# PantoMatrix/PantoMatrix

Measured on NVIDIA H100. Metric: motion_frames_per_sec, higher is better.
Workload: dtype fp16x3 (two fp16 operand planes, 3 products, f32 accumulate)

## Files before the change

### include/pm_emage.h

```cpp
#ifndef PM_EMAGE_H
#define PM_EMAGE_H
#include <stdint.h>
#ifdef __cplusplus
extern "C" {
#endif

#define PM_ABI_VERSION 6
#define PM_FMT_F16 0x100
#define PM_TC_TILE_SHIFT 16
int pm_abi_version(void);
int pm_memset_async(void* ptr, int value, long long bytes, void* stream);
int pm_device_cc(void);

int pm_tapgemm_f32(const float* A, long long a_bs, int lda, int batch, int rows_in, int cin,
                   const float* W, const float* bias, int taps, int stride, int pad,
                   int rows_out, int cout,
                   const float* residual, long long r_bs, int ldr,
                   int act, float slope,
                   float* out, long long o_bs, int ldo, void* stream);

int pm_tapgemm_tc(const uint16_t* A, long long a_ps, long long a_bs, int lda, int batch, int rows_in, int cin,
                  const uint16_t* W, long long w_ps, int w_rows, int ldw, int taps, int pad, int nsplit,
                  const float* bias, int rows_out, int cout,
                  const float* residual, long long r_bs, int ldr,
                  int act, int act_cols, float slope, float acc_scale,
                  float* out_f32, long long o_bs, int ldo,
                  uint16_t* out_bf16, long long ob_ps, long long ob_bs, int ldob, int out_nsplit,
                  const void* prefetch, long long prefetch_bytes, void* stream);

int pm_split_bf16(const float* x, long long x_bs, int ldx, int batch, int rows, int ch,
                  uint16_t* out, long long o_ps, long long o_bs, int ldo, int nsplit, void* stream);

// ... 114 lines not shown
```

### pantomatrix_b200/csrc/pm_common.cuh

```cuda
#pragma once
#include <cuda_bf16.h>
#include <cuda_fp16.h>
#include <cuda_runtime.h>
#include <stdint.h>

#define PM_OK 0
#define PM_EBADARG (-1)
#define PM_EUNSUPPORTED (-2)

#define PM_LAUNCH_CHECK()                                  \
  do {                                                     \
    cudaError_t _e = cudaGetLastError();                   \
    return _e == cudaSuccess ? PM_OK : (int)_e;            \
  } while (0)

#define PM_REQUIRE(cond) \
  do {                   \
    if (!(cond)) return PM_EBADARG; \
  } while (0)

static inline int pm_cdiv(long long a, long long b) { return (int)((a + b - 1) / b); }

static inline bool pm_first_use_on_device(unsigned long long& mask) {
  int d = 0;
// ... 37 lines not shown
  int nsplit;
};

__device__ __forceinline__ void pm_split3(float v, __nv_bfloat16 (&p)[3]) {
  p[0] = __float2bfloat16_rn(v);
  float r = v - __bfloat162float(p[0]);
  p[1] = __float2bfloat16_rn(r);
  r -= __bfloat162float(p[1]);
  p[2] = __float2bfloat16_rn(r);
}

#ifndef PM_FMT_F16
#define PM_FMT_F16 0x100
#endif
#define PM_F16_ACT_SCALE 64.0f
#define PM_TAKE_FMT(nsplit_var, flag_var)                          \
  const bool flag_var = ((nsplit_var) & PM_FMT_F16) != 0;          \
  (nsplit_var) &= 0xff

__device__ __forceinline__ float pm_f16_head(float v) {
  return __uint_as_float((__float_as_uint(v) + 0x00001000u) & 0xFFFFE000u);
}

template <bool F16>
__device__ __forceinline__ void pm_store_planes_t(const PmPlanes& P, long long row, int c, float v) {
  if constexpr (F16) {
    __half* o = reinterpret_cast<__half*>(P.ptr) + row * P.ld + c;
    v *= PM_F16_ACT_SCALE;
    if (P.nsplit <= 2) {
      const float f0 = P.nsplit == 2 ? pm_f16_head(v) : v;
      o[0] = __float2half_rn(f0);
      if (P.nsplit == 2) o[P.ps] = __float2half_rn(v - f0);
    } else {
      for (int pl = 0; pl < P.nsplit; ++pl) {
        const __half h = __float2half_rn(v);
        o[(long long)pl * P.ps] = h;
        v -= __half2float(h);
      }
    }
  } else {
    __nv_bfloat16* o = P.ptr + row * P.ld + c;
    for (int pl = 0; pl < P.nsplit; ++pl) {
      const __nv_bfloat16 h = __float2bfloat16_rn(v);
      o[(long long)pl * P.ps] = h;
      v -= __bfloat162float(h);
    }
  }
}
__device__ __forceinline__ void pm_store_planes(const PmPlanes& P, long long row, int c, float v) {
  pm_store_planes_t<false>(P, row, c, v);
}

template <bool F16>
__device__ __forceinline__ void pm_store_planes4_t(const PmPlanes& P, long long row, int c, float4 v) {
  if constexpr (F16) {
    __half* o = reinterpret_cast<__half*>(P.ptr) + row * P.ld + c;
    v.x *= PM_F16_ACT_SCALE; v.y *= PM_F16_ACT_SCALE; v.z *= PM_F16_ACT_SCALE; v.w *= PM_F16_ACT_SCALE;
    if (P.nsplit == 2) {
      const float4 f = make_float4(pm_f16_head(v.x), pm_f16_head(v.y), pm_f16_head(v.z), pm_f16_head(v.w));
      const __half2 a0 = __floats2half2_rn(f.x, f.y), a1 = __floats2half2_rn(f.z, f.w);
      const __half2 b0 = __floats2half2_rn(v.x - f.x, v.y - f.y), b1 = __floats2half2_rn(v.z - f.z, v.w - f.w);
      uint2 w0, w1;
      w0.x = *reinterpret_cast<const uint32_t*>(&a0); w0.y = *reinterpret_cast<const uint32_t*>(&a1);
      w1.x = *reinterpret_cast<const uint32_t*>(&b0); w1.y = *reinterpret_cast<const uint32_t*>(&b1);
      *reinterpret_cast<uint2*>(o) = w0;
      *reinterpret_cast<uint2*>(o + P.ps) = w1;
      return;
    }
    for (int pl = 0; pl < P.nsplit; ++pl) {
      const __half2 lo = __floats2half2_rn(v.x, v.y), hi = __floats2half2_rn(v.z, v.w);
      uint2 w;
      w.x = *reinterpret_cast<const uint32_t*>(&lo);
      w.y = *reinterpret_cast<const uint32_t*>(&hi);
      *reinterpret_cast<uint2*>(o + (long long)pl * P.ps) = w;
      v.x -= __low2float(lo); v.y -= __high2float(lo); v.z -= __low2float(hi); v.w -= __high2float(hi);
    }
  } else {
    __nv_bfloat16* o = P.ptr + row * P.ld + c;
    for (int pl = 0; pl < P.nsplit; ++pl) {
      const __nv_bfloat162 lo = __floats2bfloat162_rn(v.x, v.y), hi = __floats2bfloat162_rn(v.z, v.w);
      uint2 w;
      w.x = *reinterpret_cast<const uint32_t*>(&lo);
      w.y = *reinterpret_cast<const uint32_t*>(&hi);
      *reinterpret_cast<uint2*>(o + (long long)pl * P.ps) = w;
      v.x -= __low2float(lo); v.y -= __high2float(lo); v.z -= __low2float(hi); v.w -= __high2float(hi);
    }
  }
}
__device__ __forceinline__ void pm_store_planes4(const PmPlanes& P, long long row, int c, float4 v) {
  pm_store_planes4_t<false>(P, row, c, v);
}

static inline bool pm_planes_ok(const void* ptr, long long ps, int ld, int nsplit, int ch, bool vec4) {
  if (!ptr) return true;
  if (nsplit < 1 || nsplit > 3 || ld < ch) return false;
  if (vec4 && ((ld & 3) || (ps & 3) || (reinterpret_cast<uintptr_t>(ptr) & 7))) return false;
  return true;
}
```

### pantomatrix_b200/csrc/pm_tapgemm_tc.cu

```cuda
#include <cuda.h>
#include <stdio.h>
#include <stdlib.h>

#include <cstring>
#include "pm_common.cuh"
#include "../../include/pm_emage.h"


namespace {

constexpr int BM = 128;
constexpr int BK = 64;
constexpr int MMA_K = 16;
constexpr int A_TILE_BYTES = BM * BK * 2;
constexpr int PRODUCER_THREADS = 128;
constexpr int CONSUMER_THREADS = 256;
constexpr int NUM_THREADS = PRODUCER_THREADS + CONSUMER_THREADS;
constexpr int PRODUCER_REGS = 40, CONSUMER_REGS = 232;
static_assert(PRODUCER_THREADS * PRODUCER_REGS + CONSUMER_THREADS * CONSUMER_REGS == (65536 / NUM_THREADS & ~7) * NUM_THREADS,
              "the setmaxnreg split must use exactly the launch's register pool");
constexpr int STAMP_WARP = PRODUCER_THREADS / 32;
constexpr int MAX_STAGES = 8;
constexpr int RING_KB = 200;

struct TcParams {
  int taps, pad, nsplit, kblocks;
  int rows_out, cout, batch;
  int R, NB;
  int w_rows;
  const float* bias;
  const float* residual; long long r_bs; int ldr;
  int res_tma;
  int act, act_cols; float slope;
  float* out_f32; long long o_bs; int ldo;
  __nv_bfloat16* out_bf16; long long ob_ps, ob_bs; int ldob; int out_nsplit;
  int stages;
  int res_slot0, rot;
  const uint8_t* prefetch; long long prefetch_bytes;
  float acc_scale;
};

#ifdef PM_TC_TIMING
__device__ unsigned long long pm_tc_stamps[4096 * 8];
#define PM_STAMP(i)                                                                                              \
  do {                                                                                                           \
    if ((threadIdx.x & 31) == 0) {                                                                               \
      const unsigned cta_ = (blockIdx.z * gridDim.y + blockIdx.y) * gridDim.x + blockIdx.x;                      \
      if (cta_ < 4096) pm_tc_stamps[cta_ * 8 + (i)] = (unsigned long long)clock64();                             \
    }                                                                                                            \
  } while (0)
#else
#define PM_STAMP(i) do {} while (0)
#endif

#include "pm_tc_ptx.cuh"
// ... 10 lines not shown
  constexpr uint64_t A_PL = A_TILE_BYTES >> 4, W_PL = (BN * BK * 2) >> 4, K_ST = (MMA_K * 2) >> 4;
  if constexpr (NSPLIT == 3) {
#pragma unroll
    for (int k = 0; k < BK / MMA_K; ++k) mma_k16<BN, F16>(corr, a0 + k * K_ST, w0 + 2 * W_PL + k * K_ST);
#pragma unroll
    for (int k = 0; k < BK / MMA_K; ++k) mma_k16<BN, F16>(corr, a0 + A_PL + k * K_ST, w0 + W_PL + k * K_ST);
#pragma unroll
    for (int k = 0; k < BK / MMA_K; ++k) mma_k16<BN, F16>(corr, a0 + 2 * A_PL + k * K_ST, w0 + k * K_ST);
  }
  if constexpr (NSPLIT >= 2) {
#pragma unroll
    for (int k = 0; k < BK / MMA_K; ++k) mma_k16<BN, F16>(corr, a0 + k * K_ST, w0 + W_PL + k * K_ST);
#pragma unroll
    for (int k = 0; k < BK / MMA_K; ++k) mma_k16<BN, F16>(corr, a0 + A_PL + k * K_ST, w0 + k * K_ST);
  }
#pragma unroll
  for (int k = 0; k < BK / MMA_K; ++k) mma_k16<BN, F16>(main, a0 + k * K_ST, w0 + k * K_ST);
}

template <int BN, bool F16, int NSPLIT>
__global__ void __launch_bounds__(NUM_THREADS, 1) tapgemm_tc_kernel(const __grid_constant__ CUtensorMap map_a,
                                                                  const __grid_constant__ CUtensorMap map_w,
                                                                  const __grid_constant__ CUtensorMap map_r,
                                                                  const TcParams p) {
  constexpr int W_TILE_BYTES = BN * BK * 2;
  constexpr int NACC = BN / 2;
  constexpr int ST = BN + 8;
  constexpr int RES_BYTES = BM * BN * 4;

  extern __shared__ __align__(1024) uint8_t smem_raw[];
  uint8_t* tiles = reinterpret_cast<uint8_t*>((reinterpret_cast<uintptr_t>(smem_raw) + 1023) & ~uintptr_t(1023));
  const int stage_bytes = p.nsplit * (A_TILE_BYTES + W_TILE_BYTES);
  const int ring_bytes = p.stages * stage_bytes > BM * ST * 4 ? p.stages * stage_bytes : BM * ST * 4;
  uint64_t* bars = reinterpret_cast<uint64_t*>(tiles + ring_bytes);
  uint64_t* full_bar = bars;
  uint64_t* empty_bar = bars + MAX_STAGES;
  uint64_t* epi_bar = bars + 2 * MAX_STAGES;
  float* bias_s = reinterpret_cast<float*>(bars + 2 * MAX_STAGES + 2);

  const int warp = threadIdx.x >> 5, lane = threadIdx.x & 31;
  if (warp == STAMP_WARP) PM_STAMP(0);
  const int l0 = blockIdx.x * p.R;
  const int n0 = blockIdx.y * BN;
  const int b0 = blockIdx.z * p.NB;
  const int n_iter = p.taps * p.kblocks;

  if (threadIdx.x == 0) {
    asm volatile("prefetch.tensormap [%0];" ::"l"(&map_a) : "memory");
    asm volatile("prefetch.tensormap [%0];" ::"l"(&map_w) : "memory");
    if (p.res_tma) asm volatile("prefetch.tensormap [%0];" ::"l"(&map_r) : "memory");
    for (int s = 0; s < p.stages; ++s) {
      mbar_init(smem_u32(&full_bar[s]), 1);
      mbar_init(smem_u32(&empty_bar[s]), 2);
    }
    mbar_init(smem_u32(epi_bar), p.res_tma ? 2 : 1);
    asm volatile("fence.mbarrier_init.release.cluster;" ::: "memory");
  }
  __syncthreads();
  if (warp == STAMP_WARP) PM_STAMP(1);

  if (warp < PRODUCER_THREADS / 32) {
    setmaxnreg_dec<PRODUCER_REGS>();
    if (warp == 1 && lane == 0 && p.prefetch) {
      const long long ncta = (long long)gridDim.x * gridDim.y * gridDim.z;
      const long long cta = ((long long)blockIdx.z * gridDim.y + blockIdx.y) * gridDim.x + blockIdx.x;
      long long share = ((p.prefetch_bytes + ncta - 1) / ncta + 127) & ~127LL;
      long long off = cta * share;
      long long end = off + share < p.prefetch_bytes ? off + share : p.prefetch_bytes;
      end &= ~15LL;
      for (; off < end; off += 16384) {
        const uint32_t n = (uint32_t)(end - off < 16384 ? end - off : 16384);
        asm volatile("cp.async.bulk.prefetch.L2.global [%0], %1;" ::"l"(p.prefetch + off), "r"(n) : "memory");
      }
// ... 11 lines not shown
      mbar_wait_fast(smem_u32(&empty_bar[s]), ph ^ 1u);
      if (elect_one()) {
        const uint32_t bar = smem_u32(&full_bar[s]);
        uint8_t* st = tiles + (size_t)q * stage_bytes;
        mbar_expect_tx(bar, tx);
        for (int pl = 0; pl < p.nsplit; ++pl) {
          tma_load_4d(smem_u32(st + pl * A_TILE_BYTES), &map_a, bar, kb * BK, l0 + tap - p.pad, b0, pl);
          tma_load_3d(smem_u32(st + p.nsplit * A_TILE_BYTES + pl * W_TILE_BYTES), &map_w, bar, kb * BK, tap * p.w_rows + n0, pl);
        }
      }
      __syncwarp();
      if (++s == p.stages) { s = 0; ph ^= 1u; }
      if (++q == p.stages) q = 0;
      if (++kb == p.kblocks) { kb = 0; ++tap; }
    }
    if (p.res_tma) {
      for (int j = p.res_slot0; j < p.stages; ++j) {
        mbar_wait_fast(smem_u32(&empty_bar[s]), ph ^ 1u);
        if (++s == p.stages) { s = 0; ph ^= 1u; }
      }
      if (elect_one()) {
        const uint32_t bar = smem_u32(epi_bar);
        mbar_expect_tx(bar, (uint32_t)RES_BYTES);
        tma_load_3d(smem_u32(tiles + ring_bytes - RES_BYTES), &map_r, bar, n0, l0, b0);
      }
      __syncwarp();
    }
    return;
  }

  setmaxnreg_inc<CONSUMER_REGS>();
  const int ct = threadIdx.x - PRODUCER_THREADS;
  const int wg = ct >> 7;
  float acc0[NACC], acc1[NACC], accc[NACC];
#pragma unroll
  for (int i = 0; i < NACC; ++i) { acc0[i] = 0.f; acc1[i] = 0.f; accc[i] = 0.f; }
  {
    const uint32_t tiles_u32 = smem_u32(tiles);
    int s = 0, q = p.rot;
    uint32_t ph = 0;
    int prev = -1;
    auto kblock = [&](float (&main)[NACC]) {
      mbar_wait_fast(smem_u32(&full_bar[s]), ph);
      if (prev < 0 && warp == STAMP_WARP) PM_STAMP(2);
      const uint32_t a_base = tiles_u32 + (uint32_t)q * (uint32_t)stage_bytes + (uint32_t)wg * (64 * 128);
      const uint32_t w_base = tiles_u32 + (uint32_t)q * (uint32_t)stage_bytes + (uint32_t)(NSPLIT * A_TILE_BYTES);
      wgmma_fence();
      mma_kblock<BN, F16, NSPLIT>(main, accc, gmma_desc(GMMA_DESC_K_SW128, a_base), gmma_desc(GMMA_DESC_K_SW128, w_base));
      wgmma_commit();
      wgmma_wait<1>();
      if (prev >= 0 && ct % 128 == 0) mbar_arrive(smem_u32(&empty_bar[prev]));
      prev = s;
      if (++s == p.stages) { s = 0; ph ^= 1u; }
      if (++q == p.stages) q = 0;
    };
    int it = 0;
    for (; it + 1 < n_iter; it += 2) {
      kblock(acc0);
      kblock(acc1);
    }
    if (it < n_iter) kblock(acc0);
    if (warp == STAMP_WARP) PM_STAMP(3);
    wgmma_wait<0>();
    if (warp == STAMP_WARP) PM_STAMP(4);
    wgmma_fence_regs(acc0);
    wgmma_fence_regs(acc1);
    wgmma_fence_regs(accc);
  }
  named_bar_sync(1, CONSUMER_THREADS);
  {
    const int wq = warp & 3, t4 = lane & 3;
    const int r0 = wg * 64 + wq * 16 + (lane >> 2);
    float* stg = reinterpret_cast<float*>(tiles);
#pragma unroll
    for (int i = 0; i < NACC / 4; ++i) {
      const int c = 8 * i + 2 * t4;
#pragma unroll
      for (int h = 0; h < 2; ++h) {
        float v0 = acc0[4 * i + 2 * h] + acc1[4 * i + 2 * h];
        float v1 = acc0[4 * i + 2 * h + 1] + acc1[4 * i + 2 * h + 1];
        v0 += accc[4 * i + 2 * h];
        v1 += accc[4 * i + 2 * h + 1];
        if constexpr (F16) { v0 *= p.acc_scale; v1 *= p.acc_scale; }
        *reinterpret_cast<float2*>(stg + (r0 + 8 * h) * ST + c) = make_float2(v0, v1);
      }
    }
  }
  named_bar_sync(1, CONSUMER_THREADS);

  const bool vec_f = p.out_f32 && ((p.ldo & 3) == 0) && ((reinterpret_cast<uintptr_t>(p.out_f32) & 15) == 0) && ((p.o_bs & 3) == 0);
  const bool vec_b = p.out_bf16 && ((p.ldob & 3) == 0) && ((reinterpret_cast<uintptr_t>(p.out_bf16) & 7) == 0) &&
                     ((p.ob_bs & 3) == 0) && ((p.ob_ps & 3) == 0);
// ... 58 lines not shown
                                                         long long o_bs, int ldo, int nsplit) {
  const int b = blockIdx.y;
  const float* __restrict__ xb = x + (long long)b * x_bs;
  __nv_bfloat16* __restrict__ ob = out + (long long)b * o_bs;
  if (VEC) {
    const int ch4 = ch >> 2;
    const long long total = (long long)rows * ch4;
    for (long long i = (long long)blockIdx.x * blockDim.x + threadIdx.x; i < total; i += (long long)gridDim.x * blockDim.x) {
      const int r = (int)(i / ch4), c4 = (int)(i - (long long)r * ch4);
      const float4 v = *reinterpret_cast<const float4*>(xb + (long long)r * ldx + 4 * c4);
      const PmPlanes P{ob, o_ps, ldo, nsplit};
      pm_store_planes4_t<F16>(P, r, 4 * c4, v);
    }
  } else {
    const long long total = (long long)rows * ch;
    for (long long i = (long long)blockIdx.x * blockDim.x + threadIdx.x; i < total; i += (long long)gridDim.x * blockDim.x) {
      const int r = (int)(i / ch), c = (int)(i - (long long)r * ch);
      const PmPlanes P{ob, o_ps, ldo, nsplit};
      pm_store_planes_t<F16>(P, r, c, xb[(long long)r * ldx + c]);
    }
  }
}

template <int BN, bool F16, int NSPLIT>
int launch(const CUtensorMap& ma, const CUtensorMap& mw, const CUtensorMap& mr, TcParams& p, dim3 grid, cudaStream_t st) {
  constexpr int stage_bytes = NSPLIT * (A_TILE_BYTES + BN * BK * 2);
  constexpr int stages = RING_KB * 1024 / stage_bytes < MAX_STAGES ? RING_KB * 1024 / stage_bytes : MAX_STAGES;
  static_assert(stages >= 2, "the operand ring needs two stages");
  constexpr int staging = BM * (BN + 8) * 4, res_bytes = BM * BN * 4;
  static_assert(staging + res_bytes <= stages * stage_bytes && res_bytes <= (stages - 1) * stage_bytes,
                "staging and residual tiles must fit the ring side by side");
  p.stages = stages;
  p.res_slot0 = (stages * stage_bytes - res_bytes) / stage_bytes;
  p.rot = (p.res_slot0 - 1 - (p.taps * p.kblocks - 1) % stages + stages) % stages;
  const size_t smem = (size_t)stages * stage_bytes + 1024  + (2 * MAX_STAGES + 2) * sizeof(uint64_t) + BN * sizeof(float);
  static unsigned long long configured = 0;
  if (pm_first_use_on_device(configured)) {
    cudaError_t e = cudaFuncSetAttribute(tapgemm_tc_kernel<BN, F16, NSPLIT>, cudaFuncAttributeMaxDynamicSharedMemorySize, 227 * 1024);
    if (e != cudaSuccess) { configured = 0; return (int)e; }
  }
  tapgemm_tc_kernel<BN, F16, NSPLIT><<<grid, NUM_THREADS, smem, st>>>(ma, mw, mr, p);
  PM_LAUNCH_CHECK();
}

template <int BN>
int launch_fmt(const CUtensorMap& ma, const CUtensorMap& mw, const CUtensorMap& mr, TcParams& p, dim3 grid, cudaStream_t st,
               bool f16) {
  if (f16) {
    if (p.nsplit == 1) return launch<BN, true, 1>(ma, mw, mr, p, grid, st);
    if (p.nsplit == 2) return launch<BN, true, 2>(ma, mw, mr, p, grid, st);
    return launch<BN, true, 3>(ma, mw, mr, p, grid, st);
  }
  if (p.nsplit == 1) return launch<BN, false, 1>(ma, mw, mr, p, grid, st);
  if (p.nsplit == 2) return launch<BN, false, 2>(ma, mw, mr, p, grid, st);
  return launch<BN, false, 3>(ma, mw, mr, p, grid, st);
}

int pick_bn(long long row_tiles, int cout, int w_rows, int sms) {
  if (cout <= 64 || w_rows % 128) return 64;
  const long long waves64 = (row_tiles * pm_cdiv(cout, 64) + sms - 1) / sms;
  const long long waves128 = (row_tiles * pm_cdiv(cout, 128) + sms - 1) / sms;
  return waves128 * 14 <= waves64 * 10 ? 128 : 64;
}

}

extern "C" int pm_tapgemm_tc(const uint16_t* A, long long a_ps, long long a_bs, int lda, int batch, int rows_in, int cin,
                             const uint16_t* W, long long w_ps, int w_rows, int ldw, int taps, int pad, int nsplit,
                             const float* bias, int rows_out, int cout,
                             const float* residual, long long r_bs, int ldr,
                             int act, int act_cols, float slope, float acc_scale,
                             float* out_f32, long long o_bs, int ldo,
                             uint16_t* out_bf16, long long ob_ps, long long ob_bs, int ldob, int out_nsplit,
                             const void* prefetch, long long prefetch_bytes, void* stream) {
  PM_REQUIRE(A && W && (out_f32 || out_bf16));
  const int tile = (nsplit >> PM_TC_TILE_SHIFT) & 0xff;
  PM_TAKE_FMT(nsplit, f16);
  PM_TAKE_FMT(out_nsplit, out_f16);
  PM_REQUIRE(!out_bf16 || out_f16 == f16);
  PM_REQUIRE(f16 || acc_scale == 1.0f);
  PM_REQUIRE(!prefetch || (prefetch_bytes >= 0 && (reinterpret_cast<uintptr_t>(prefetch) & 15) == 0));
  PM_REQUIRE(batch > 0 && rows_in > 0 && rows_out > 0 && cin > 0 && cout > 0 && taps > 0);
  PM_REQUIRE(nsplit >= 1 && nsplit <= 3 && (!out_bf16 || (out_nsplit >= 1 && out_nsplit <= 3)));
  PM_REQUIRE(act >= PM_ACT_NONE && act <= PM_ACT_LEAKY);
  PM_REQUIRE((reinterpret_cast<uintptr_t>(A) & 15) == 0 && (reinterpret_cast<uintptr_t>(W) & 15) == 0);
  PM_REQUIRE((lda & 7) == 0 && (ldw & 7) == 0 && lda >= cin && ldw >= cin && w_rows >= cout);
  PM_REQUIRE(batch == 1 || (a_bs & 7) == 0);
  PM_REQUIRE(nsplit == 1 || ((a_ps & 7) == 0 && (w_ps & 7) == 0));
  PM_REQUIRE(!out_f32 || ldo >= cout);
  PM_REQUIRE(!out_bf16 || ldob >= cout);
  PM_REQUIRE(!residual || ldr >= cout);

  int R = 128;
  if (rows_out <= 64 && batch > 1) { R = 16; while (R < rows_out) R <<= 1; }
  const int NB = 128 / R;
  PM_REQUIRE(tile <= 2 && w_rows % 64 == 0 && (tile != 2 || w_rows % 128 == 0));
  int BNsel = tile == 1 ? 64 : 128;
  if (tile == 0) {
    int dev = 0, sms = 0;
    cudaError_t e = cudaGetDevice(&dev);
    if (e == cudaSuccess) e = cudaDeviceGetAttribute(&sms, cudaDevAttrMultiProcessorCount, dev);
    if (e != cudaSuccess) return (int)e;
    BNsel = pick_bn((long long)pm_cdiv(rows_out, R) * pm_cdiv(batch, NB), cout, w_rows, sms);
  }

  TcParams p;
  p.taps = taps; p.pad = pad; p.nsplit = nsplit; p.kblocks = (cin + BK - 1) / BK;
  p.rows_out = rows_out; p.cout = cout; p.batch = batch; p.R = R; p.NB = NB; p.w_rows = w_rows;
  p.bias = bias; p.residual = residual; p.r_bs = r_bs; p.ldr = ldr;
  p.act = act; p.act_cols = act_cols <= 0 ? cout : act_cols; p.slope = slope;
  p.out_f32 = out_f32; p.o_bs = o_bs; p.ldo = ldo;
  p.out_bf16 = reinterpret_cast<__nv_bfloat16*>(out_bf16); p.ob_ps = ob_ps; p.ob_bs = ob_bs; p.ldob = ldob;
  p.out_nsplit = out_bf16 ? out_nsplit : 0;
  p.stages = 0;
  p.prefetch = static_cast<const uint8_t*>(prefetch);
  p.prefetch_bytes = prefetch ? prefetch_bytes : 0;
  p.acc_scale = acc_scale;
  CUtensorMap ma, mw;
  {
    const long long bs_el = batch > 1 ? a_bs : (long long)rows_in * lda;
    const long long ps_el = nsplit > 1 ? a_ps : bs_el * batch;
    cuuint64_t dims[4] = {(cuuint64_t)cin, (cuuint64_t)rows_in, (cuuint64_t)batch, (cuuint64_t)nsplit};
    cuuint64_t strides[3] = {(cuuint64_t)lda * 2, (cuuint64_t)bs_el * 2, (cuuint64_t)ps_el * 2};
    cuuint32_t box[4] = {(cuuint32_t)BK, (cuuint32_t)R, (cuuint32_t)NB, 1};
    if (!encode_map(&ma, A, 4, dims, strides, box, f16)) return PM_EBADARG;
  }
  {
    const long long ps_el = nsplit > 1 ? w_ps : (long long)taps * w_rows * ldw;
    cuuint64_t dims[3] = {(cuuint64_t)cin, (cuuint64_t)taps * w_rows, (cuuint64_t)nsplit};
    cuuint64_t strides[2] = {(cuuint64_t)ldw * 2, (cuuint64_t)ps_el * 2};
    cuuint32_t box[3] = {(cuuint32_t)BK, (cuuint32_t)BNsel, 1};
    if (!encode_map(&mw, W, 3, dims, strides, box, f16)) return PM_EBADARG;
  }
  CUtensorMap mr;
  std::memset(&mr, 0, sizeof(mr));
  p.res_tma = residual && (reinterpret_cast<uintptr_t>(residual) & 15) == 0 && (ldr & 3) == 0 && (batch == 1 || (r_bs & 3) == 0);
  if (p.res_tma) {
    const long long bs_el = batch > 1 ? r_bs : (long long)rows_out * ldr;
    cuuint64_t dims[3] = {(cuuint64_t)cout, (cuuint64_t)rows_out, (cuuint64_t)batch};
    cuuint64_t strides[2] = {(cuuint64_t)ldr * 4, (cuuint64_t)bs_el * 4};
    cuuint32_t box[3] = {(cuuint32_t)BNsel, (cuuint32_t)R, (cuuint32_t)NB};
    p.res_tma = encode_tiled(&mr, CU_TENSOR_MAP_DATA_TYPE_FLOAT32, CU_TENSOR_MAP_SWIZZLE_NONE, residual, 3, dims, strides, box);
  }
  dim3 grid(pm_cdiv(rows_out, R), pm_cdiv(cout, BNsel), pm_cdiv(batch, NB));
  PM_REQUIRE(grid.z <= 65535 && grid.y <= 65535);
  const cudaStream_t st = (cudaStream_t)stream;
  if (BNsel == 128) return launch_fmt<128>(ma, mw, mr, p, grid, st, f16);
  return launch_fmt<64>(ma, mw, mr, p, grid, st, f16);
}

#ifdef PM_TC_TIMING
extern "C" int pm_tc_timing_reset() {
  cudaError_t e = cudaDeviceSynchronize();
  if (e != cudaSuccess) return (int)e;
  void* d = nullptr;
  e = cudaGetSymbolAddress(&d, pm_tc_stamps);
  if (e != cudaSuccess) return (int)e;
  return (int)cudaMemset(d, 0, sizeof(unsigned long long) * 4096 * 8);
}
extern "C" int pm_tc_timing_read(unsigned long long* host) {
  cudaError_t e = cudaDeviceSynchronize();
  if (e != cudaSuccess) return (int)e;
  return (int)cudaMemcpyFromSymbol(host, pm_tc_stamps, sizeof(unsigned long long) * 4096 * 8);
}
#endif

extern "C" int pm_split_bf16(const float* x, long long x_bs, int ldx, int batch, int rows, int ch,
                             uint16_t* out, long long o_ps, long long o_bs, int ldo, int nsplit, void* stream) {
  PM_TAKE_FMT(nsplit, f16);
  PM_REQUIRE(x && out && batch >= 0 && rows >= 0 && ch > 0 && ldx >= ch && ldo >= ch && nsplit >= 1 && nsplit <= 3);
  if ((long long)batch * rows == 0) return PM_OK;
// ... 20 lines not shown
```

### pantomatrix_b200/csrc/pm_tc_ptx.cuh

```cuda
#pragma once
#include <cuda.h>
#include <stdint.h>

__device__ __forceinline__ uint32_t smem_u32(const void* p) { return (uint32_t)__cvta_generic_to_shared(p); }

__device__ __forceinline__ void mbar_init(uint32_t bar, uint32_t count) {
  asm volatile("mbarrier.init.shared::cta.b64 [%0], %1;" ::"r"(bar), "r"(count) : "memory");
}
__device__ __forceinline__ void mbar_expect_tx(uint32_t bar, uint32_t bytes) {
  asm volatile("mbarrier.arrive.expect_tx.shared::cta.b64 _, [%0], %1;" ::"r"(bar), "r"(bytes) : "memory");
}
static __device__ __noinline__ void pm_watchdog_trap() { __trap(); }
__device__ __forceinline__ void mbar_wait(uint32_t bar, uint32_t parity) {
  uint32_t spins = 0;
  long long t0 = 0;
  while (true) {
    uint32_t done;
    asm volatile(
        "{\n\t.reg .pred p;\n\t"
        "mbarrier.try_wait.parity.shared::cta.b64 p, [%1], %2;\n\t"
        "selp.u32 %0, 1, 0, p;\n\t}"
        : "=r"(done) : "r"(bar), "r"(parity) : "memory");
    if (done) return;
    if ((++spins & 0xFFFu) == 0) {
// ... 22 lines not shown
  uint32_t done;
  asm volatile(
      "{\n\t.reg .pred p;\n\t"
      "mbarrier.try_wait.parity.shared::cta.b64 p, [%1], %2;\n\t"
      "selp.u32 %0, 1, 0, p;\n\t}"
      : "=r"(done) : "r"(bar), "r"(parity) : "memory");
  if (!done) mbar_wait(bar, parity);
}
__device__ __forceinline__ bool elect_one() {
  uint32_t pred;
  asm volatile("{\n\t.reg .pred P1;\n\telect.sync _|P1, 0xffffffff;\n\tselp.u32 %0, 1, 0, P1;\n\t}" : "=r"(pred));
  return pred != 0;
}
__device__ __forceinline__ void tma_load_4d(uint32_t dst, const CUtensorMap* map, uint32_t bar, int c0, int c1, int c2, int c3) {
  asm volatile(
      "cp.async.bulk.tensor.4d.shared::cluster.global.mbarrier::complete_tx::bytes [%0], [%1, {%3, %4, %5, %6}], [%2];"
      ::"r"(dst), "l"(map), "r"(bar), "r"(c0), "r"(c1), "r"(c2), "r"(c3) : "memory");
}
__device__ __forceinline__ void tma_load_3d(uint32_t dst, const CUtensorMap* map, uint32_t bar, int c0, int c1, int c2) {
  asm volatile(
      "cp.async.bulk.tensor.3d.shared::cluster.global.mbarrier::complete_tx::bytes [%0], [%1, {%3, %4, %5}], [%2];"
      ::"r"(dst), "l"(map), "r"(bar), "r"(c0), "r"(c1), "r"(c2) : "memory");
}
__device__ __forceinline__ void sts128(uint32_t addr, float a, float b, float c, float d) {
  asm volatile("st.shared.v4.f32 [%0], {%1, %2, %3, %4};" ::"r"(addr), "f"(a), "f"(b), "f"(c), "f"(d) : "memory");
}
__device__ __forceinline__ float4 lds128(uint32_t addr) {
  float4 v;
  asm volatile("ld.shared.v4.f32 {%0, %1, %2, %3}, [%4];" : "=f"(v.x), "=f"(v.y), "=f"(v.z), "=f"(v.w) : "r"(addr) : "memory");
  return v;
}
__device__ __forceinline__ void mbar_arrive(uint32_t bar) {
  asm volatile("mbarrier.arrive.shared::cta.b64 _, [%0];" ::"r"(bar) : "memory");
}
__device__ __forceinline__ void fence_proxy_async_smem() { asm volatile("fence.proxy.async.shared::cta;" ::: "memory"); }
__device__ __forceinline__ float4 ldg_stream4(const float4* p) {
  float4 v;
  asm volatile("ld.global.nc.L1::no_allocate.v4.f32 {%0, %1, %2, %3}, [%4];"
               : "=f"(v.x), "=f"(v.y), "=f"(v.z), "=f"(v.w) : "l"(p));
  return v;
}
template <int N>
__device__ __forceinline__ void setmaxnreg_dec() { asm volatile("setmaxnreg.dec.sync.aligned.u32 %0;" ::"n"(N)); }
template <int N>
__device__ __forceinline__ void setmaxnreg_inc() { asm volatile("setmaxnreg.inc.sync.aligned.u32 %0;" ::"n"(N)); }
__device__ __forceinline__ void named_bar_sync(uint32_t id, uint32_t threads) {
// ... 98 lines not shown
```

### pantomatrix_b200/ops.py

```python
from __future__ import annotations

import math

import torch

from . import _lib

ACT_NONE, ACT_RELU, ACT_LEAKY = 0, 1, 2
ROW_NONE, ROW_PE, ROW_SPK = 0, 1, 2

launch_count = 0

FMT_F16 = 0x100
TC_TILE_SHIFT = 16
F16_ACT_SCALE = 64.0
_PLANE_DTYPE = torch.bfloat16


def set_plane_format(name: str) -> None:
    global _PLANE_DTYPE
    _PLANE_DTYPE = {"bf16": torch.bfloat16, "fp16": torch.float16}[name]


def plane_format() -> str:
    return "fp16" if _PLANE_DTYPE == torch.float16 else "bf16"


def _fmt_bit(t) -> int:
    return FMT_F16 if t.dtype == torch.float16 else 0


def _stream() -> int:
    return torch.cuda.current_stream().cuda_stream


def _ptr(t) -> int | None:
    return None if t is None else t.data_ptr()
# ... 381 lines not shown
        taps, cout, cin = w.shape
        bn = 64 if cout <= 64 else 128
        self.taps, self.cout, self.cin = taps, cout, cin
        self.w_rows, self.ldw = _round_up(cout, bn), _round_up(cin, 8)
        full = torch.zeros(taps, self.w_rows, self.ldw, device=w.device, dtype=torch.float32)
        full[:, :cout, :cin] = w
        self.acc_scale = 1.0
        if _PLANE_DTYPE == torch.float16:
            m = float(full.abs().max())
            if m > 0.0 and math.isfinite(m):
                k = math.floor(math.log2(32768.0 / m))
                full = full * (2.0 ** k)
                self.acc_scale = 2.0 ** -k
            self.acc_scale /= F16_ACT_SCALE
        planes, rem = [], full
        for _ in range(nsplit):
            p = rem.to(_PLANE_DTYPE)
            planes.append(p)
            rem = rem - p.float()
        self.t = torch.stack(planes).contiguous()


def tapgemm_tc(a: Planes, w: PackedW, bias, *, rows_in=None, rows_out, pad=0, act=ACT_NONE, act_cols=0, slope=0.0,
               residual=None, want_f32=True, out_nsplit=0, out=None, a_view=None, out_slack=0, prefetch=None, tile=0):
    t = a.t
    nsplit, batch = t.shape[0], t.shape[1]
    assert nsplit == w.t.shape[0] and t.dtype == w.t.dtype, "A and W must use the same split and plane format"
    fmt = _fmt_bit(t)
    rows_a, cin, lda = (a.rows, a.ch, t.stride(2)) if a_view is None else a_view
    if rows_in is not None:
        rows_a = rows_in
    assert cin == w.cin, (cin, w.cin)
    assert tile in (0, 64, 128), tile
    cout = w.cout
    dev = t.device
    out_f = None
    if want_f32:
        out_f = out if out is not None else torch.empty(batch, rows_out, cout, device=dev, dtype=torch.float32)
        assert out_f.shape == (batch, rows_out, cout)
    o_bs, ldo = _bs_ld(out_f) if out_f is not None else (0, 0)
    out_p = None
    if out_nsplit:
        out_p = _new_planes(out_nsplit, (batch, rows_out), cout, dev, out_slack, dtype=t.dtype)
    r_bs, ldr = _bs_ld(residual) if residual is not None else (0, 0)
    if residual is not None:
        _chk(residual)
        assert residual.shape == (batch, rows_out, cout)
    _call("pm_tapgemm_tc", t.data_ptr(), t.stride(0), t.stride(1), lda, batch, rows_a, cin,
          w.t.data_ptr(), w.t.stride(0), w.w_rows, w.ldw, w.taps, pad, nsplit | fmt | (tile // 64) << TC_TILE_SHIFT,
          _ptr(bias), rows_out, cout, _ptr(residual), r_bs, ldr, act, act_cols, float(slope), float(w.acc_scale),
          _ptr(out_f), o_bs, ldo,
          None if out_p is None else out_p.t.data_ptr(), 0 if out_p is None else out_p.t.stride(0),
          0 if out_p is None else out_p.t.stride(1), 0 if out_p is None else out_p.t.stride(2),
          out_nsplit | (fmt if out_nsplit else 0),
          None if prefetch is None else prefetch.data_ptr(),
          0 if prefetch is None else prefetch.numel() * prefetch.element_size(), _stream())
    return out_f, out_p




def lstm_bidir(xproj, whh, barrier, hidden):
    _chk(xproj), _chk(whh)
    assert xproj.is_contiguous() and whh.is_contiguous() and whh.shape == (2, 4 * hidden, hidden)
    batch, t, w = xproj.shape
    assert w == 8 * hidden
    y = torch.empty(batch, t, 2 * hidden, device=xproj.device, dtype=torch.float32)
    _call("pm_lstm_bidir_f32", xproj.data_ptr(), xproj.stride(0), xproj.stride(1), whh.data_ptr(), y.data_ptr(),
          y.stride(0), y.stride(1), barrier.data_ptr(), batch, t, hidden, _stream())
    return y


# ... 156 lines not shown
```

Baseline: 326,000.

## Store tapgemm epilogue through swizzled shared memory with TMA bulk tensor stores

```diff
diff --git a/include/pm_emage.h b/include/pm_emage.h
--- a/include/pm_emage.h
+++ b/include/pm_emage.h
@@ -8,6 +8,7 @@
 #define PM_ABI_VERSION 6
 #define PM_FMT_F16 0x100
 #define PM_TC_TILE_SHIFT 16
+#define PM_TC_STORE_LOOP (1 << 24)
 int pm_abi_version(void);
 int pm_memset_async(void* ptr, int value, long long bytes, void* stream);
 int pm_device_cc(void);
diff --git a/pantomatrix_b200/csrc/pm_common.cuh b/pantomatrix_b200/csrc/pm_common.cuh
--- a/pantomatrix_b200/csrc/pm_common.cuh
+++ b/pantomatrix_b200/csrc/pm_common.cuh
@@ -83,30 +83,47 @@
   return __uint_as_float((__float_as_uint(v) + 0x00001000u) & 0xFFFFE000u);
 }
 
-template <bool F16>
-__device__ __forceinline__ void pm_store_planes_t(const PmPlanes& P, long long row, int c, float v) {
+template <bool F16, int NS = 0>
+__device__ __forceinline__ void pm_split_pair_t(float x, float y, int nsplit, uint32_t (&w)[3]) {
+  if constexpr (NS > 0) nsplit = NS;
   if constexpr (F16) {
-    __half* o = reinterpret_cast<__half*>(P.ptr) + row * P.ld + c;
-    v *= PM_F16_ACT_SCALE;
-    if (P.nsplit <= 2) {
-      const float f0 = P.nsplit == 2 ? pm_f16_head(v) : v;
-      o[0] = __float2half_rn(f0);
-      if (P.nsplit == 2) o[P.ps] = __float2half_rn(v - f0);
-    } else {
-      for (int pl = 0; pl < P.nsplit; ++pl) {
-        const __half h = __float2half_rn(v);
-        o[(long long)pl * P.ps] = h;
-        v -= __half2float(h);
+    x = __fmul_rn(x, PM_F16_ACT_SCALE);
+    y = __fmul_rn(y, PM_F16_ACT_SCALE);
+    if (nsplit == 2) {
+      const float fx = pm_f16_head(x), fy = pm_f16_head(y);
+      const __half2 a = __floats2half2_rn(fx, fy), b = __floats2half2_rn(x - fx, y - fy);
+      w[0] = *reinterpret_cast<const uint32_t*>(&a);
+      w[1] = *reinterpret_cast<const uint32_t*>(&b);
+      return;
+    }
+#pragma unroll
+    for (int pl = 0; pl < 3; ++pl) {
+      if (pl < nsplit) {
+        const __half2 h = __floats2half2_rn(x, y);
+        w[pl] = *reinterpret_cast<const uint32_t*>(&h);
+        x -= __low2float(h); y -= __high2float(h);
       }
     }
   } else {
-    __nv_bfloat16* o = P.ptr + row * P.ld + c;
-    for (int pl = 0; pl < P.nsplit; ++pl) {
-      const __nv_bfloat16 h = __float2bfloat16_rn(v);
-      o[(long long)pl * P.ps] = h;
-      v -= __bfloat162float(h);
+#pragma unroll
+    for (int pl = 0; pl < 3; ++pl) {
+      if (pl < nsplit) {
+        const __nv_bfloat162 h = __floats2bfloat162_rn(x, y);
+        w[pl] = *reinterpret_cast<const uint32_t*>(&h);
+        x -= __low2float(h); y -= __high2float(h);
+      }
     }
   }
+}
+
+template <bool F16>
+__device__ __forceinline__ void pm_store_planes_t(const PmPlanes& P, long long row, int c, float v) {
+  uint16_t* o = reinterpret_cast<uint16_t*>(P.ptr) + row * P.ld + c;
+  uint32_t w[3];
+  pm_split_pair_t<F16>(v, 0.f, P.nsplit, w);
+#pragma unroll
+  for (int pl = 0; pl < 3; ++pl)
+    if (pl < P.nsplit) o[(long long)pl * P.ps] = (uint16_t)w[pl];
 }
 __device__ __forceinline__ void pm_store_planes(const PmPlanes& P, long long row, int c, float v) {
   pm_store_planes_t<false>(P, row, c, v);
@@ -114,39 +131,13 @@
 
 template <bool F16>
 __device__ __forceinline__ void pm_store_planes4_t(const PmPlanes& P, long long row, int c, float4 v) {
-  if constexpr (F16) {
-    __half* o = reinterpret_cast<__half*>(P.ptr) + row * P.ld + c;
-    v.x *= PM_F16_ACT_SCALE; v.y *= PM_F16_ACT_SCALE; v.z *= PM_F16_ACT_SCALE; v.w *= PM_F16_ACT_SCALE;
-    if (P.nsplit == 2) {
-      const float4 f = make_float4(pm_f16_head(v.x), pm_f16_head(v.y), pm_f16_head(v.z), pm_f16_head(v.w));
-      const __half2 a0 = __floats2half2_rn(f.x, f.y), a1 = __floats2half2_rn(f.z, f.w);
-      const __half2 b0 = __floats2half2_rn(v.x - f.x, v.y - f.y), b1 = __floats2half2_rn(v.z - f.z, v.w - f.w);
-      uint2 w0, w1;
-      w0.x = *reinterpret_cast<const uint32_t*>(&a0); w0.y = *reinterpret_cast<const uint32_t*>(&a1);
-      w1.x = *reinterpret_cast<const uint32_t*>(&b0); w1.y = *reinterpret_cast<const uint32_t*>(&b1);
-      *reinterpret_cast<uint2*>(o) = w0;
-      *reinterpret_cast<uint2*>(o + P.ps) = w1;
-      return;
-    }
-    for (int pl = 0; pl < P.nsplit; ++pl) {
-      const __half2 lo = __floats2half2_rn(v.x, v.y), hi = __floats2half2_rn(v.z, v.w);
-      uint2 w;
-      w.x = *reinterpret_cast<const uint32_t*>(&lo);
-      w.y = *reinterpret_cast<const uint32_t*>(&hi);
-      *reinterpret_cast<uint2*>(o + (long long)pl * P.ps) = w;
-      v.x -= __low2float(lo); v.y -= __high2float(lo); v.z -= __low2float(hi); v.w -= __high2float(hi);
-    }
-  } else {
-    __nv_bfloat16* o = P.ptr + row * P.ld + c;
-    for (int pl = 0; pl < P.nsplit; ++pl) {
-      const __nv_bfloat162 lo = __floats2bfloat162_rn(v.x, v.y), hi = __floats2bfloat162_rn(v.z, v.w);
-      uint2 w;
-      w.x = *reinterpret_cast<const uint32_t*>(&lo);
-      w.y = *reinterpret_cast<const uint32_t*>(&hi);
-      *reinterpret_cast<uint2*>(o + (long long)pl * P.ps) = w;
-      v.x -= __low2float(lo); v.y -= __high2float(lo); v.z -= __low2float(hi); v.w -= __high2float(hi);
-    }
-  }
+  __nv_bfloat16* o = P.ptr + row * P.ld + c;
+  uint32_t lo[3], hi[3];
+  pm_split_pair_t<F16>(v.x, v.y, P.nsplit, lo);
+  pm_split_pair_t<F16>(v.z, v.w, P.nsplit, hi);
+#pragma unroll
+  for (int pl = 0; pl < 3; ++pl)
+    if (pl < P.nsplit) *reinterpret_cast<uint2*>(o + (long long)pl * P.ps) = make_uint2(lo[pl], hi[pl]);
 }
 __device__ __forceinline__ void pm_store_planes4(const PmPlanes& P, long long row, int c, float4 v) {
   pm_store_planes4_t<false>(P, row, c, v);
diff --git a/pantomatrix_b200/csrc/pm_tapgemm_tc.cu b/pantomatrix_b200/csrc/pm_tapgemm_tc.cu
--- a/pantomatrix_b200/csrc/pm_tapgemm_tc.cu
+++ b/pantomatrix_b200/csrc/pm_tapgemm_tc.cu
@@ -3,6 +3,7 @@
 #include <stdlib.h>
 
 #include <cstring>
+#include <type_traits>
 #include "pm_common.cuh"
 #include "../../include/pm_emage.h"
 
@@ -31,6 +32,7 @@
   const float* bias;
   const float* residual; long long r_bs; int ldr;
   int res_tma;
+  int tma_out;
   int act, act_cols; float slope;
   float* out_f32; long long o_bs; int ldo;
   __nv_bfloat16* out_bf16; long long ob_ps, ob_bs; int ldob; int out_nsplit;
@@ -87,6 +89,8 @@
 __global__ void __launch_bounds__(NUM_THREADS, 1) tapgemm_tc_kernel(const __grid_constant__ CUtensorMap map_a,
                                                                   const __grid_constant__ CUtensorMap map_w,
                                                                   const __grid_constant__ CUtensorMap map_r,
+                                                                  const __grid_constant__ CUtensorMap map_o,
+                                                                  const __grid_constant__ CUtensorMap map_p,
                                                                   const TcParams p) {
   constexpr int W_TILE_BYTES = BN * BK * 2;
   constexpr int NACC = BN / 2;
@@ -94,7 +98,7 @@
   constexpr int RES_BYTES = BM * BN * 4;
 
   extern __shared__ __align__(1024) uint8_t smem_raw[];
-  uint8_t* tiles = reinterpret_cast<uint8_t*>((reinterpret_cast<uintptr_t>(smem_raw) + 1023) & ~uintptr_t(1023));
+  uint8_t* tiles = smem_raw + ((1024u - (smem_u32(smem_raw) & 1023u)) & 1023u);
   const int stage_bytes = p.nsplit * (A_TILE_BYTES + W_TILE_BYTES);
   const int ring_bytes = p.stages * stage_bytes > BM * ST * 4 ? p.stages * stage_bytes : BM * ST * 4;
   uint64_t* bars = reinterpret_cast<uint64_t*>(tiles + ring_bytes);
@@ -114,6 +118,8 @@
     asm volatile("prefetch.tensormap [%0];" ::"l"(&map_a) : "memory");
     asm volatile("prefetch.tensormap [%0];" ::"l"(&map_w) : "memory");
     if (p.res_tma) asm volatile("prefetch.tensormap [%0];" ::"l"(&map_r) : "memory");
+    if (p.tma_out && p.out_f32) asm volatile("prefetch.tensormap [%0];" ::"l"(&map_o) : "memory");
+    if (p.tma_out && p.out_nsplit) asm volatile("prefetch.tensormap [%0];" ::"l"(&map_p) : "memory");
     for (int s = 0; s < p.stages; ++s) {
       mbar_init(smem_u32(&full_bar[s]), 1);
       mbar_init(smem_u32(&empty_bar[s]), 2);
@@ -171,7 +177,9 @@
       if (elect_one()) {
         const uint32_t bar = smem_u32(epi_bar);
         mbar_expect_tx(bar, (uint32_t)RES_BYTES);
-        tma_load_3d(smem_u32(tiles + ring_bytes - RES_BYTES), &map_r, bar, n0, l0, b0);
+        const int nbox = p.tma_out ? BN / 32 : 1;
+        for (int j = 0; j < nbox; ++j)
+          tma_load_3d(smem_u32(tiles + ring_bytes - RES_BYTES + j * (RES_BYTES / nbox)), &map_r, bar, n0 + j * (BN / nbox), l0, b0);
       }
       __syncwarp();
     }
@@ -217,6 +225,81 @@
     wgmma_fence_regs(accc);
   }
   named_bar_sync(1, CONSUMER_THREADS);
+  if (p.tma_out) {
+    const int wq = warp & 3, t4 = lane & 3, sw = lane >> 2;
+    const int r0 = wg * 64 + wq * 16 + sw;
+    const float act_slope = p.act == PM_ACT_NONE ? 1.f : (p.act == PM_ACT_RELU ? 0.f : p.slope);
+    const float* res_s = reinterpret_cast<const float*>(tiles + ring_bytes - RES_BYTES);
+    auto off32 = [&](int r, int i) { return (i >> 2) * (BM * 32) + r * 32 + (((2 * (i & 3) + (t4 >> 1)) ^ sw) << 2) + 2 * (t4 & 1); };
+    mbar_wait_fast(smem_u32(epi_bar), 0);
+#pragma unroll
+    for (int i = 0; i < NACC / 4; ++i) {
+      const int c = 8 * i + 2 * t4, n = n0 + c;
+      const float2 bc = *reinterpret_cast<const float2*>(bias_s + c);
+#pragma unroll
+      for (int h = 0; h < 2; ++h) {
+        const int j = 4 * i + 2 * h;
+        float v0 = acc0[j] + acc1[j], v1 = acc0[j + 1] + acc1[j + 1];
+        v0 += accc[j];
+        v1 += accc[j + 1];
+        if constexpr (F16) { v0 = __fmul_rn(v0, p.acc_scale); v1 = __fmul_rn(v1, p.acc_scale); }
+        if (p.bias) { v0 += bc.x; v1 += bc.y; }
+        if (p.residual) {
+          const float2 t = *reinterpret_cast<const float2*>(res_s + off32(r0 + 8 * h, i));
+          v0 += t.x; v1 += t.y;
+        }
+        acc0[j] = v0 < 0.f ? (n < p.act_cols ? act_slope : 1.f) * v0 : v0;
+        acc0[j + 1] = v1 < 0.f ? (n + 1 < p.act_cols ? act_slope : 1.f) * v1 : v1;
+      }
+    }
+    float* of_s = reinterpret_cast<float*>(tiles);
+    uint8_t* pl_s = tiles + (p.out_f32 ? BM * BN * 4 : 0);
+    constexpr int PLANE_BYTES = BM * BN * 2;
+    if (p.out_f32) {
+#pragma unroll
+      for (int i = 0; i < NACC / 4; ++i)
+#pragma unroll
+        for (int h = 0; h < 2; ++h)
+          *reinterpret_cast<float2*>(of_s + off32(r0 + 8 * h, i)) = make_float2(acc0[4 * i + 2 * h], acc0[4 * i + 2 * h + 1]);
+      fence_proxy_async_smem();
+      named_bar_sync(1, CONSUMER_THREADS);
+      if (ct == 0) {
+        for (int j = 0; j < BN / 32 && n0 + 32 * j < p.cout; ++j)
+          tma_store_3d(&map_o, smem_u32(of_s + j * (BM * 32)), n0 + 32 * j, l0, b0);
+        bulk_commit();
+      }
+    }
+    auto planes = [&](auto ons) {
+      constexpr int ONS = decltype(ons)::value;
+#pragma unroll
+      for (int i = 0; i < NACC / 4; ++i)
+#pragma unroll
+        for (int h = 0; h < 2; ++h) {
+          uint32_t w[3];
+          pm_split_pair_t<F16, ONS>(acc0[4 * i + 2 * h], acc0[4 * i + 2 * h + 1], p.out_nsplit, w);
+          const int o = (i >> 3) * (BM * 128) + (r0 + 8 * h) * 128 + (((i & 7) ^ sw) << 4) + 4 * t4;
+#pragma unroll
+          for (int pl = 0; pl < 3; ++pl)
+            if (pl < (ONS ? ONS : p.out_nsplit)) *reinterpret_cast<uint32_t*>(pl_s + pl * PLANE_BYTES + o) = w[pl];
+        }
+    };
+    if (p.out_nsplit) {
+      if (p.out_nsplit == NSPLIT) planes(std::integral_constant<int, NSPLIT>{});
+      else planes(std::integral_constant<int, 0>{});
+      fence_proxy_async_smem();
+      named_bar_sync(1, CONSUMER_THREADS);
+      if (ct == 0) {
+        for (int pl = 0; pl < p.out_nsplit; ++pl)
+          for (int j = 0; j < BN / 64 && n0 + 64 * j < p.cout; ++j)
+            tma_store_4d(&map_p, smem_u32(pl_s + pl * PLANE_BYTES + j * (BM * 128)), n0 + 64 * j, l0, b0, pl);
+        bulk_commit();
+      }
+    }
+    if (warp == STAMP_WARP) PM_STAMP(5);
+    if (ct == 0) bulk_wait_read0();
+    if (warp == STAMP_WARP) PM_STAMP(6);
+    return;
+  }
   {
     const int wq = warp & 3, t4 = lane & 3;
     const int r0 = wg * 64 + wq * 16 + (lane >> 2);
@@ -321,14 +404,26 @@
   }
 }
 
+constexpr int stage_bytes_of(int bn, int nsplit) { return nsplit * (A_TILE_BYTES + bn * BK * 2); }
+constexpr int stages_of(int bn, int nsplit) {
+  return RING_KB * 1024 / stage_bytes_of(bn, nsplit) < MAX_STAGES ? RING_KB * 1024 / stage_bytes_of(bn, nsplit) : MAX_STAGES;
+}
+constexpr int ring_bytes_of(int bn, int nsplit) { return stages_of(bn, nsplit) * stage_bytes_of(bn, nsplit); }
+constexpr bool tma_out_fits(int bn, int nsplit, bool f32, int out_nsplit, bool residual) {
+  return (f32 ? BM * bn * 4 : 0) + out_nsplit * BM * bn * 2 + (residual ? BM * bn * 4 : 0) <= ring_bytes_of(bn, nsplit);
+}
+
 template <int BN, bool F16, int NSPLIT>
-int launch(const CUtensorMap& ma, const CUtensorMap& mw, const CUtensorMap& mr, TcParams& p, dim3 grid, cudaStream_t st) {
-  constexpr int stage_bytes = NSPLIT * (A_TILE_BYTES + BN * BK * 2);
-  constexpr int stages = RING_KB * 1024 / stage_bytes < MAX_STAGES ? RING_KB * 1024 / stage_bytes : MAX_STAGES;
+int launch(const CUtensorMap& ma, const CUtensorMap& mw, const CUtensorMap& mr, const CUtensorMap& mo,
+           const CUtensorMap& mp, TcParams& p, dim3 grid, cudaStream_t st) {
+  constexpr int stage_bytes = stage_bytes_of(BN, NSPLIT);
+  constexpr int stages = stages_of(BN, NSPLIT);
   static_assert(stages >= 2, "the operand ring needs two stages");
   constexpr int staging = BM * (BN + 8) * 4, res_bytes = BM * BN * 4;
   static_assert(staging + res_bytes <= stages * stage_bytes && res_bytes <= (stages - 1) * stage_bytes,
                 "staging and residual tiles must fit the ring side by side");
+  static_assert(tma_out_fits(BN, NSPLIT, true, 2, true), "fp32, two plane and residual tiles must fit the ring");
+  static_assert(BN * 4 * BM % 1024 == 0 && stage_bytes % 1024 == 0, "128B-swizzled TMA boxes need 1024-byte alignment");
   p.stages = stages;
   p.res_slot0 = (stages * stage_bytes - res_bytes) / stage_bytes;
   p.rot = (p.res_slot0 - 1 - (p.taps * p.kblocks - 1) % stages + stages) % stages;
@@ -338,21 +433,20 @@
     cudaError_t e = cudaFuncSetAttribute(tapgemm_tc_kernel<BN, F16, NSPLIT>, cudaFuncAttributeMaxDynamicSharedMemorySize, 227 * 1024);
     if (e != cudaSuccess) { configured = 0; return (int)e; }
   }
-  tapgemm_tc_kernel<BN, F16, NSPLIT><<<grid, NUM_THREADS, smem, st>>>(ma, mw, mr, p);
+  tapgemm_tc_kernel<BN, F16, NSPLIT><<<grid, NUM_THREADS, smem, st>>>(ma, mw, mr, mo, mp, p);
   PM_LAUNCH_CHECK();
 }
 
 template <int BN>
-int launch_fmt(const CUtensorMap& ma, const CUtensorMap& mw, const CUtensorMap& mr, TcParams& p, dim3 grid, cudaStream_t st,
-               bool f16) {
+int launch_fmt(const CUtensorMap* m, TcParams& p, dim3 grid, cudaStream_t st, bool f16) {
   if (f16) {
-    if (p.nsplit == 1) return launch<BN, true, 1>(ma, mw, mr, p, grid, st);
-    if (p.nsplit == 2) return launch<BN, true, 2>(ma, mw, mr, p, grid, st);
-    return launch<BN, true, 3>(ma, mw, mr, p, grid, st);
-  }
-  if (p.nsplit == 1) return launch<BN, false, 1>(ma, mw, mr, p, grid, st);
-  if (p.nsplit == 2) return launch<BN, false, 2>(ma, mw, mr, p, grid, st);
-  return launch<BN, false, 3>(ma, mw, mr, p, grid, st);
+    if (p.nsplit == 1) return launch<BN, true, 1>(m[0], m[1], m[2], m[3], m[4], p, grid, st);
+    if (p.nsplit == 2) return launch<BN, true, 2>(m[0], m[1], m[2], m[3], m[4], p, grid, st);
+    return launch<BN, true, 3>(m[0], m[1], m[2], m[3], m[4], p, grid, st);
+  }
+  if (p.nsplit == 1) return launch<BN, false, 1>(m[0], m[1], m[2], m[3], m[4], p, grid, st);
+  if (p.nsplit == 2) return launch<BN, false, 2>(m[0], m[1], m[2], m[3], m[4], p, grid, st);
+  return launch<BN, false, 3>(m[0], m[1], m[2], m[3], m[4], p, grid, st);
 }
 
 int pick_bn(long long row_tiles, int cout, int w_rows, int sms) {
@@ -374,6 +468,7 @@
                              const void* prefetch, long long prefetch_bytes, void* stream) {
   PM_REQUIRE(A && W && (out_f32 || out_bf16));
   const int tile = (nsplit >> PM_TC_TILE_SHIFT) & 0xff;
+  const bool store_loop = (nsplit & PM_TC_STORE_LOOP) != 0;
   PM_TAKE_FMT(nsplit, f16);
   PM_TAKE_FMT(out_nsplit, out_f16);
   PM_REQUIRE(!out_bf16 || out_f16 == f16);
@@ -415,7 +510,9 @@
   p.prefetch = static_cast<const uint8_t*>(prefetch);
   p.prefetch_bytes = prefetch ? prefetch_bytes : 0;
   p.acc_scale = acc_scale;
-  CUtensorMap ma, mw;
+  CUtensorMap m[5];
+  std::memset(m, 0, sizeof(m));
+  CUtensorMap &ma = m[0], &mw = m[1], &mr = m[2], &mo = m[3], &mp = m[4];
   {
     const long long bs_el = batch > 1 ? a_bs : (long long)rows_in * lda;
     const long long ps_el = nsplit > 1 ? a_ps : bs_el * batch;
@@ -431,21 +528,42 @@
     cuuint32_t box[3] = {(cuuint32_t)BK, (cuuint32_t)BNsel, 1};
     if (!encode_map(&mw, W, 3, dims, strides, box, f16)) return PM_EBADARG;
   }
-  CUtensorMap mr;
-  std::memset(&mr, 0, sizeof(mr));
-  p.res_tma = residual && (reinterpret_cast<uintptr_t>(residual) & 15) == 0 && (ldr & 3) == 0 && (batch == 1 || (r_bs & 3) == 0);
-  if (p.res_tma) {
+  const bool res_ok = residual && (reinterpret_cast<uintptr_t>(residual) & 15) == 0 && (ldr & 3) == 0 && (batch == 1 || (r_bs & 3) == 0);
+  bool tma_out = !store_loop && (!residual || res_ok) && tma_out_fits(BNsel, nsplit, out_f32, p.out_nsplit, residual);
+  if (tma_out && out_f32) {
+    tma_out = (reinterpret_cast<uintptr_t>(out_f32) & 15) == 0 && (ldo & 3) == 0 && (batch == 1 || (o_bs & 3) == 0);
+    const long long bs_el = batch > 1 ? o_bs : (long long)rows_out * ldo;
+    cuuint64_t dims[3] = {(cuuint64_t)cout, (cuuint64_t)rows_out, (cuuint64_t)batch};
+    cuuint64_t strides[2] = {(cuuint64_t)ldo * 4, (cuuint64_t)bs_el * 4};
+    cuuint32_t box[3] = {32, (cuuint32_t)R, (cuuint32_t)NB};
+    tma_out = tma_out && encode_tiled(&mo, CU_TENSOR_MAP_DATA_TYPE_FLOAT32, CU_TENSOR_MAP_SWIZZLE_128B, out_f32, 3, dims, strides, box);
+  }
+  if (tma_out && out_bf16) {
+    tma_out = (reinterpret_cast<uintptr_t>(out_bf16) & 15) == 0 && (ldob & 7) == 0 && (batch == 1 || (ob_bs & 7) == 0) &&
+              (out_nsplit == 1 || (ob_ps & 7) == 0);
+    const long long bs_el = batch > 1 ? ob_bs : (long long)rows_out * ldob;
+    const long long ps_el = out_nsplit > 1 ? ob_ps : bs_el * batch;
+    cuuint64_t dims[4] = {(cuuint64_t)cout, (cuuint64_t)rows_out, (cuuint64_t)batch, (cuuint64_t)out_nsplit};
+    cuuint64_t strides[3] = {(cuuint64_t)ldob * 2, (cuuint64_t)bs_el * 2, (cuuint64_t)ps_el * 2};
+    cuuint32_t box[4] = {64, (cuuint32_t)R, (cuuint32_t)NB, 1};
+    tma_out = tma_out && encode_map(&mp, out_bf16, 4, dims, strides, box, f16);
+  }
+  p.res_tma = false;
+  for (int swz = tma_out; res_ok && !p.res_tma && swz >= 0; --swz) {
     const long long bs_el = batch > 1 ? r_bs : (long long)rows_out * ldr;
     cuuint64_t dims[3] = {(cuuint64_t)cout, (cuuint64_t)rows_out, (cuuint64_t)batch};
     cuuint64_t strides[2] = {(cuuint64_t)ldr * 4, (cuuint64_t)bs_el * 4};
-    cuuint32_t box[3] = {(cuuint32_t)BNsel, (cuuint32_t)R, (cuuint32_t)NB};
-    p.res_tma = encode_tiled(&mr, CU_TENSOR_MAP_DATA_TYPE_FLOAT32, CU_TENSOR_MAP_SWIZZLE_NONE, residual, 3, dims, strides, box);
-  }
+    cuuint32_t box[3] = {swz ? 32u : (cuuint32_t)BNsel, (cuuint32_t)R, (cuuint32_t)NB};
+    p.res_tma = encode_tiled(&mr, CU_TENSOR_MAP_DATA_TYPE_FLOAT32, swz ? CU_TENSOR_MAP_SWIZZLE_128B : CU_TENSOR_MAP_SWIZZLE_NONE,
+                             residual, 3, dims, strides, box);
+    if (!p.res_tma) tma_out = false;
+  }
+  p.tma_out = tma_out;
   dim3 grid(pm_cdiv(rows_out, R), pm_cdiv(cout, BNsel), pm_cdiv(batch, NB));
   PM_REQUIRE(grid.z <= 65535 && grid.y <= 65535);
   const cudaStream_t st = (cudaStream_t)stream;
-  if (BNsel == 128) return launch_fmt<128>(ma, mw, mr, p, grid, st, f16);
-  return launch_fmt<64>(ma, mw, mr, p, grid, st, f16);
+  if (BNsel == 128) return launch_fmt<128>(m, p, grid, st, f16);
+  return launch_fmt<64>(m, p, grid, st, f16);
 }
 
 #ifdef PM_TC_TIMING
diff --git a/pantomatrix_b200/csrc/pm_tc_ptx.cuh b/pantomatrix_b200/csrc/pm_tc_ptx.cuh
--- a/pantomatrix_b200/csrc/pm_tc_ptx.cuh
+++ b/pantomatrix_b200/csrc/pm_tc_ptx.cuh
@@ -68,6 +68,16 @@
       "cp.async.bulk.tensor.3d.shared::cluster.global.mbarrier::complete_tx::bytes [%0], [%1, {%3, %4, %5}], [%2];"
       ::"r"(dst), "l"(map), "r"(bar), "r"(c0), "r"(c1), "r"(c2) : "memory");
 }
+__device__ __forceinline__ void tma_store_3d(const CUtensorMap* map, uint32_t src, int c0, int c1, int c2) {
+  asm volatile("cp.async.bulk.tensor.3d.global.shared::cta.bulk_group [%0, {%2, %3, %4}], [%1];"
+               ::"l"(map), "r"(src), "r"(c0), "r"(c1), "r"(c2) : "memory");
+}
+__device__ __forceinline__ void tma_store_4d(const CUtensorMap* map, uint32_t src, int c0, int c1, int c2, int c3) {
+  asm volatile("cp.async.bulk.tensor.4d.global.shared::cta.bulk_group [%0, {%2, %3, %4, %5}], [%1];"
+               ::"l"(map), "r"(src), "r"(c0), "r"(c1), "r"(c2), "r"(c3) : "memory");
+}
+__device__ __forceinline__ void bulk_commit() { asm volatile("cp.async.bulk.commit_group;" ::: "memory"); }
+__device__ __forceinline__ void bulk_wait_read0() { asm volatile("cp.async.bulk.wait_group.read 0;" ::: "memory"); }
 __device__ __forceinline__ void sts128(uint32_t addr, float a, float b, float c, float d) {
   asm volatile("st.shared.v4.f32 [%0], {%1, %2, %3, %4};" ::"r"(addr), "f"(a), "f"(b), "f"(c), "f"(d) : "memory");
 }
diff --git a/pantomatrix_b200/ops.py b/pantomatrix_b200/ops.py
--- a/pantomatrix_b200/ops.py
+++ b/pantomatrix_b200/ops.py
@@ -13,6 +13,7 @@
 
 FMT_F16 = 0x100
 TC_TILE_SHIFT = 16
+TC_STORE_LOOP = 1 << 24
 F16_ACT_SCALE = 64.0
 _PLANE_DTYPE = torch.bfloat16
 
@@ -440,7 +441,8 @@
 
 
 def tapgemm_tc(a: Planes, w: PackedW, bias, *, rows_in=None, rows_out, pad=0, act=ACT_NONE, act_cols=0, slope=0.0,
-               residual=None, want_f32=True, out_nsplit=0, out=None, a_view=None, out_slack=0, prefetch=None, tile=0):
+               residual=None, want_f32=True, out_nsplit=0, out=None, a_view=None, out_slack=0, prefetch=None, tile=0,
+               store_loop=False):
     t = a.t
     nsplit, batch = t.shape[0], t.shape[1]
     assert nsplit == w.t.shape[0] and t.dtype == w.t.dtype, "A and W must use the same split and plane format"
@@ -465,7 +467,7 @@
         _chk(residual)
         assert residual.shape == (batch, rows_out, cout)
     _call("pm_tapgemm_tc", t.data_ptr(), t.stride(0), t.stride(1), lda, batch, rows_a, cin,
-          w.t.data_ptr(), w.t.stride(0), w.w_rows, w.ldw, w.taps, pad, nsplit | fmt | (tile // 64) << TC_TILE_SHIFT,
+          w.t.data_ptr(), w.t.stride(0), w.w_rows, w.ldw, w.taps, pad, nsplit | fmt | (tile // 64) << TC_TILE_SHIFT | (TC_STORE_LOOP if store_loop else 0),
           _ptr(bias), rows_out, cout, _ptr(residual), r_bs, ldr, act, act_cols, float(slope), float(w.acc_scale),
           _ptr(out_f), o_bs, ldo,
           None if out_p is None else out_p.t.data_ptr(), 0 if out_p is None else out_p.t.stride(0),
```

After: 341,100, median of 6. +4.6%, better.
